# cyrillefavreau/Sol-R

Hardware: AMD Instinct MI355X
Metric: Mrays/s @1920x1080, 3-bounce Cornell (higher is better)
Workload: dtype f32; 1 GPU; cornell 1920x1080, 3 bounces + shadow rays, 75 boxes / 29 primitives, one GPU, whole frame; rays_per_frame=6518779, closest_hit_walks_rank0=3506171, lane_nodes=206382796, lane_prim_tests=37557299, wave_nodes=3396811, wave_prim_tests=626627, wave_walks=106204, cost_ordered_launch_rank0=True, frames_in_flight=3, setup_frames_before_warmup=48, frames_delivered=9105, order_free_nodes=46, short_ray_lists=1, gather=none (one GPU), strips=equal rows, parallelism=tile1

## Files before the change

### sol-r_amd/csrc/engine.h

```cpp
#ifndef SOLR_ENGINE_H
#define SOLR_ENGINE_H

#include <hip/hip_runtime.h>

#include <atomic>
#include <chrono>
#include <cstdio>
#include <cstdlib>
#include <cstring>
#include <string>
#include <vector>

#include "../../include/solr_hip.h"
#include "renderer.h"
#include "lists_device.h"
#include "list_builders.h"

namespace solreng
{
struct HostProfile
{
    const bool on = getenv("SOLR_HIP_HOST_PROFILE") != nullptr;
    struct Entry
    {
// ... 165 lines not shown
    unsigned *hostStats = nullptr;
    unsigned *hostStatsDev = nullptr;
    long key[6] = {0, 0, 0, 0, 0, 0};
    int frames = 0;
    bool reorder = false;
    bool orderValid = false;
    BandCuts orderCuts = {};
    void reset()
    {
        frames = 0;
        reorder = false;
        orderValid = false;
    }
    void release();
};

enum Variant
{
    VARIANT_AUTOMATIC = 0,
    VARIANT_EXACT_LIST = 3,
    VARIANT_ALL_FEATURES = 4,
    VARIANT_NO_GROUPING = 5,
    VARIANT_NO_ORDER_FREE = 6,
    VARIANT_STACK_IN_LDS = 7,
    VARIANT_REFERENCE_LEAVES = 8,
    VARIANT_AO_FIXED_STRIDE = 9,
    VARIANT_NAN_DEEP_STACK = 10,
    VARIANT_UNSORTED_LISTS = 12,
    VARIANT_NO_BAND_WORDS = 13,
    VARIANT_ZERO_STREAM_COUNTERS = 14,
    VARIANT_NO_LAMP_CUTOFF = 15,
    VARIANT_ALL_TRIPS = 16,
    VARIANT_UPLOADED_BUILD_BOXES = 17,
    VARIANT_UPLOADED_SPHERE_LEAVES = 18
};

__host__ __device__ inline int primitiveKind(int type, int facts)
{
    if (!(facts & PRIM_FAST0))
        return KIND_GENERAL;
    if (type == ptSphere && !(facts & PRIM_PROCEDURAL))
        return KIND_SPHERE;
    if ((type == ptXYPlane || type == ptYZPlane || type == ptXZPlane) && !(facts & (PRIM_TEXTURED | PRIM_WIRE2)) &&
        !(type == ptYZPlane && (facts & PRIM_EMISSIVE)))
        return type == ptXYPlane ? KIND_PLANE_XY : (type == ptYZPlane ? KIND_PLANE_YZ : KIND_PLANE_XZ);
    if (type == ptTriangle)
        return KIND_TRIANGLE;
    if (type == ptCylinder || type == ptCone)
        return KIND_CYLINDER;
    return KIND_GENERAL;
}
__host__ __device__ inline int primitiveTag(int type, int facts, bool noKinds)
{
    return type | facts | ((noKinds ? (int)KIND_GENERAL : primitiveKind(type, facts)) << PRIM_KIND_SHIFT);
}
inline bool primitiveContained(int type, int facts)
{
    return type == ptTriangle || type == ptCylinder || (type == ptSphere && !(facts & PRIM_PROCEDURAL)) || type == ptXYPlane ||
           type == ptYZPlane || type == ptXZPlane;
}
inline bool primitiveShadowOpaque(int type, int facts)
{
    return !(facts & PRIM_TRANSPARENT) && !(facts & PRIM_TEXTURED) && type != ptCamera;
}
inline int primitiveFeatures(int type, int facts)
{
    int features = (facts & PRIM_TEXTURED) ? F_TEX : 0;
    switch (type)
    {
    case ptSphere:
    case ptEnvironment:
        return features | ((facts & PRIM_PROCEDURAL) ? F_PROC : F_SPHERE);
    case ptCylinder:
    case ptCone:
        return features | F_CYL;
    case ptEllipsoid:
        return features | F_ELL;
    case ptTriangle:
        return features | F_TRI;
    case ptCamera:
        return features | F_PLANE | F_TEX;
    default:
        return features | F_PLANE;
    }
}

struct NodeList
{
    int copies, lists;
    explicit NodeList(int copies_ = 1, int lists_ = 1) : copies(copies_), lists(lists_) {}
    std::vector<float4> rows;
    std::vector<int> start, origin;
    int nb = 0;
    unsigned offRows = 0, offLeaf = 0;
    unsigned offStart = 0;
    int ordered = 0;
    bool tight = false;
    std::vector<int> refitLevels;

    void reset() { *this = NodeList(copies, lists); }
    unsigned nodes() const { return (unsigned)lists * (unsigned)nb; }
    unsigned rowsOf(int list) const { return solrdev::listRows(offRows, (unsigned)nb, (unsigned)list); }
    unsigned offThin() const { return solrdev::listThin(offRows, nodes()); }
    unsigned offSorted() const { return solrdev::listSorted(offRows, nodes()); }
    unsigned layRows(unsigned row)
    {
        offRows = row;
        return row + (unsigned)copies * solrdev::listCopyRows(nodes());
    }
    unsigned layStart(unsigned row)
    {
        offStart = row * 4;
        return row + (nodes() + 3u) / 4u;
    }
    unsigned layLeaf(unsigned row)
    {
        row = (row + 3u) & ~3u;
        offLeaf = row;
        return row + 4u * nodes() + 4u;
    }
};


struct Arena
{
    DeviceBuffer geometry;
    unsigned offPrims = 0, offLights = 0;
    unsigned rowsFixed = 0;
    bool geometryDirty = true;
    bool deviceAhead = false;
    void layOutAgain() { geometryDirty = true; }
};
struct OrderFreeState
{
    int freeCountdown = 0;
    bool freeHostValid = true;
    bool freeDirty = false;
// ... 33 lines not shown
    bool edited = false;
    DeviceBuffer materialSets;
    int nbDeviceMaterialSets = 0;
    bool materialsSet = false;
};
enum MorphSlot
{
    MORPH_SLOT_FIRST = SOLR_MORPH_TRACK_MAX_KEYS,
    MORPH_SLOT_LAST,
    MORPH_SLOTS
};
struct MorphKey
{
    DeviceBuffer planes;
    int nbPrimitives = -1;
};
struct MorphLampAnswer
{
    int slotA, slotB;
    bool moves;
};
struct Morph
{
    MorphKey keys[MORPH_SLOTS];
    int nbTrackKeys = 0;
    std::vector<MorphLampAnswer> lampAnswers;
    long lampChecked = -1;
    DeviceBuffer lampFlag;
    int nbDeviceMorphs = 0;
    int nbDeviceTrackMorphs = 0;
};
struct Scene
{
    NodeList exact = NodeList(1, 1), walk = NodeList(2, 1), orderFree = NodeList(3, solrdev::ORDER_FREE_LISTS);
    std::vector<float4> hostPrims;
    int nbPrimitives = 0;
    DeviceBuffer lamps;
    int nbLamps = 0;
    int nested = 1;
    bool walkEncloses = false;
    OrderFreeState lists;
    Rotation rotation;
    Morph morph;
    long retags = 0;
    Arena arena;

    void newGeometry(int nested_, bool walkEncloses_, int freeCountdown_)
    {
        nested = nested_;
        walkEncloses = walkEncloses_;
        rotation.refitReady = false;
        rotation.exactStale = false;
        rotation.refitPlanPending = true;
        rotation.nbMovable = -1;
        rotation.lampMoved = false;
        rotation.edited = false;
        rotation.materialsSet = false;
        morphKeysDropped();
        arena.deviceAhead = false;
        orderFree.reset();
        lists.freeCountdown = freeCountdown_;
        lists.freeHostValid = true;
        lists.freeDirty = false;
        lists.dropStage(true);
        lists.freeStale = false;
    }
    bool orderFreeDue() { return lists.freeCountdown > 0 && --lists.freeCountdown == 0; }
// ... 538 lines not shown
```

### sol-r_amd/csrc/renderer_kernel.h

```cpp
#ifndef SOLR_RENDERER_KERNEL_H
#define SOLR_RENDERER_KERNEL_H

#include "renderer.h"

using namespace solrdev;

template <int COUNT, int FEAT, bool VOLUME = false>
#ifndef SOLR_GENERIC_WAVES
#define SOLR_GENERIC_WAVES 0
#endif
#ifndef SOLR_WAVES_PER_EU
#define SOLR_WAVES_PER_EU 4
#endif
__global__ __launch_bounds__(WAVE, (SOLR_GENERIC_WAVES && (FEAT & F_TEX)) ? SOLR_GENERIC_WAVES : SOLR_WAVES_PER_EU) void k_standardRenderer(const SceneArgs, const FrameArgs,
                                                           PixelRecord *__restrict__,
                                                           int4 *__restrict__, unsigned char *__restrict__,
                                                           unsigned long long *__restrict__)
{
    extern __shared__ float ldsStack[];
    constexpr int ARGS = FEAT | F_ARGS;
    constexpr int TRACE = (FEAT & (F_TRI | F_TEX)) ? FEAT : ARGS;
    const RendererArgs &A = rendererArgs();
    const FrameArgs &F = A.F;
    const Scene &S = A.scene();
// ... 383 lines not shown
            }
        }
    }
}

template <int FEAT>
__global__ __launch_bounds__(WAVE, SOLR_WAVES_PER_EU) void k_walkBound(const SceneArgs SA, const char *__restrict__ records,
                                                                       unsigned *__restrict__ visits, unsigned *__restrict__ skipped)
{
    extern __shared__ float ldsStack[];
    const Scene S = makeScene(SA);
    const int lane = threadIdx.x;
    const char *slot = records + (size_t)blockIdx.x * SOLR_WALK_SLOT_BYTES;
    const int4 *head = (const int4 *)slot;
    const float4 *rays = (const float4 *)(slot + 16 * (SOLR_WALK_SLOTS + 1));
    const int recorded = __builtin_amdgcn_readfirstlane(head[0].x);
    const int walks = recorded < SOLR_WALK_SLOTS ? recorded : SOLR_WALK_SLOTS;
    unsigned entries = 0;
    int left_out = recorded - walks;
    for (int j = 0; j < walks; ++j)
    {
        const int4 h = head[1 + j];
        const int kind = __builtin_amdgcn_readfirstlane(h.x);
        if (kind == WALK_GENERAL)
        {
            ++left_out;
            continue;
        }
        const float4 a = rays[((size_t)j * 64 + lane) * 2], b = rays[((size_t)j * 64 + lane) * 2 + 1];
        const int doneAfter = __float_as_int(b.w);
        const bool took_part = doneAfter >= 0;
        const WalkRay r = makeWalkRay(V(a.x, a.y, a.z), took_part ? V(b.x, b.y, b.z) : V(1.f, 1.f, 1.f));
        const int order = (FEAT & F_DEEP) ? (__builtin_amdgcn_readfirstlane(h.w) >> 1) & 3 : 0;
        const Scene W = walkList(S, __builtin_amdgcn_readfirstlane(h.y) != 0, __builtin_amdgcn_readfirstlane(h.z),
                                 (__builtin_amdgcn_readfirstlane(h.w) & 1) != 0, order != 0);
        const PackedRay pr = packRay(r);
        const float cutOff = a.w;
        int cursor = took_part ? 0 : SOLR_CURSOR_DONE;
        int cur = 0, visit = 0;
        while (cur < W.nbBoxes)
        {
            if (ballot(cursor != SOLR_CURSOR_DONE) == 0ull)
                break;
            int nbPrimitives;
            bool entered;
            int leaf;
            if ((FEAT & F_DEEP) && order == 1)
                leaf = advanceTidyDeepSorted(W, pr, cutOff, cursor, cur, nbPrimitives, entered);
            else if ((FEAT & F_DEEP) && order == 2)
                leaf = advanceTidyDeepReversed(W, pr, cutOff, cursor, cur, nbPrimitives, entered);
            else
                leaf = advanceTidy<FEAT>(W, pr, cutOff, cursor, cur, nbPrimitives, entered);
            if (leaf < 0)
                break;
            ++visit;
            entries += entered ? 1u : 0u;
            if (doneAfter == visit)
                cursor = SOLR_CURSOR_DONE;
        }
    }
    visits[(size_t)blockIdx.x * WAVE + lane] = entries;
    if (lane == 0 && left_out > 0)
        atomicAdd(skipped, (unsigned)left_out);
}

#endif
```

### sol-r_amd/csrc/rt_device.h

```cpp
#pragma once

#include <hip/hip_runtime.h>
#include "pow_table.h"

#include "../../include/solr_types.h"
#include "scene_layout.h"

namespace solrdev
{
#define SOLR_DEV __device__ __forceinline__

struct v3
{
    float x, y, z;
};

SOLR_DEV v3 V(float x, float y, float z)
{
    v3 r;
    r.x = x;
    r.y = y;
    r.z = z;
    return r;
}
// ... 837 lines not shown
#define SOLR_NOW() __builtin_readcyclecounter()
#else
#define SOLR_T(...)
#endif

template <int COUNT>
SOLR_DEV void countAdd(unsigned int &c, unsigned int v)
{
    if (COUNT == 1)
        c += v;
}

SOLR_DEV int waveMinInt(int v)
{
#pragma unroll
    for (int off = 32; off > 0; off >>= 1)
    {
        int o = __shfl_xor(v, off, 64);
        v = o < v ? o : v;
    }
    return v;
}

#define SOLR_CURSOR_DONE 0x7fffffff

#define SOLR_WALK_SLOTS 16
#define SOLR_WALK_SLOT_BYTES (16 * (SOLR_WALK_SLOTS + 1) + SOLR_WALK_SLOTS * 64 * 32)
enum WalkKind
{
    WALK_CLOSEST = 0,
    WALK_SHADOW = 1,
    WALK_GENERAL = 2
};
SOLR_DEV void recordWalk(Counters &cnt, int kind, bool freeList, int octant, bool took_part, const WalkRay &r, float cutOff,
                         int doneAfter, bool tight = false, int order = 0)
{
    const unsigned j = cnt.ordinal++;
    if (j >= SOLR_WALK_SLOTS || !cnt.record)
        return;
    const int lane = (int)threadIdx.x & 63;
    float4 *lanes = (float4 *)(cnt.record + 16 * (SOLR_WALK_SLOTS + 1)) + ((size_t)j * 64 + lane) * 2;
    lanes[0] = make_float4(r.o.x, r.o.y, r.o.z, cutOff);
    lanes[1] = make_float4(r.d.x, r.d.y, r.d.z, __int_as_float(took_part ? doneAfter : -1));
    if (lane == 0)
        ((int4 *)cnt.record)[1 + j] = make_int4(kind, freeList ? 1 : 0, octant, (tight ? 1 : 0) | (order << 1));
}

template <int FEAT>
SOLR_DEV bool extendedGeometry(const SceneInfo &si);
struct PrimRec
{
    Row2 head;
    float4 c, d;
    int pi;
    bool packed;
};
SOLR_DEV bool planeClass(int type)
{
    return !(type == ptSphere || type == ptEnvironment || type == ptCylinder || type == ptCone || type == ptEllipsoid ||
             type == ptTriangle);
}
SOLR_DEV v3 recP1(const Scene &S, const PrimRec &r) { return r.packed ? V4(r.c) : V4(primRow(S, r.pi, ROW_P1_INDEX)); }
SOLR_DEV v3 recP2(const Scene &S, const PrimRec &r) { return r.packed ? V4(r.d) : V4(primRow(S, r.pi, ROW_P2)); }
SOLR_DEV v3 recPlaneNormal(const Scene &S, const PrimRec &r) { return r.packed ? V4(r.c) : V4(primRow(S, r.pi, ROW_N0)); }
SOLR_DEV float recPlaneAverage(const Scene &S, const PrimRec &r) { return r.packed ? r.d.x : primRow(S, r.pi, ROW_P2).w; }
SOLR_DEV int recIndex(const Scene &S, const PrimRec &r)
// ... 788 lines not shown
        return 0.f;
    const Scene S = again<FEAT>(S_);
    const SceneInfo si = again<FEAT>(si_);
    SOLR_T(const unsigned long long tw0 = SOLR_NOW();)
    WalkRay r = makeWalkRay(origin, lampCenter - origin);
    r.o = origin + r.dn * si.rayEpsilon;
    const float minDistance = (iteration < 2) ? si.viewDistance : si.viewDistance / (iteration + 1);
    const float lengthOL = length(r.d);
    if (active)
        countAdd<COUNT>(cnt.shadow, 1);
    countAdd<COUNT>(cnt.wShadow, 1);

    const bool fastBoxes = S.orderedBoxes && (ballot(active && !finiteRay(r)) == 0ull);
    const bool tidy = COUNT != 1 && fastBoxes && S.nested;
    const bool freeOrder = tidy && S.nbBoxesFree > 0 && (S.opaqueShadows & SHADOWS_OPAQUE) &&
                           ballot(active && !(longRay(r.d) && minDistance >= 2.f)) == 0ull;
    const bool lampCut = tidy && !freeOrder && (S.opaqueShadows & SHADOWS_LAMP_CUTOFF);
    float farFree = 0.f;
    int octant = 0;
    bool reversed = false;
    if (freeOrder)
    {
        const int signs = ((r.d.x < 0.f ? 1 : 0) | (r.d.y < 0.f ? 2 : 0) | (r.d.z < 0.f ? 4 : 0)) ^ 7;
        const int lane = (int)__builtin_ctzll(ballot(active));
        octant = __builtin_amdgcn_readlane(signs, lane);
        reversed = (FEAT & F_DEEP) && S.sortedLists && ballot(active && signs != octant) == 0ull;
    }
    if (freeOrder || lampCut)
        farFree = 1.0002f + 1.0e-4f * (fabsf(r.o.x) + fabsf(r.o.y) + fabsf(r.o.z)) / lengthOL;
    const float farOrdered =
        (lampCut && longRay(r.d) && minDistance >= 2.f) ? fminf(minDistance, farFree) : minDistance;
    const bool tight = (FEAT & F_PLANE) && tidy && S.tightLists && ballot(active && !tightRay(r, si)) == 0ull;
    reversed = reversed && !tight;
    const Scene W = walkList(S, freeOrder, octant, tight, reversed);
    const int nbBoxes = W.nbBoxes;
    const PackedRay pr = packRay(r);
    int cursor = (active && result < si.shadowIntensity) ? 0 : SOLR_CURSOR_DONE;
    const bool walked = cursor != SOLR_CURSOR_DONE;
    int visit = 0, doneAfter = SOLR_CURSOR_DONE;
    int cur = 0;
    Row2 node;
    node.a = node.b = make_float4(0.f, 0.f, 0.f, 0.f);
    if (!tidy)
        node = boxNode(S, 0);
    while (cur < nbBoxes)
    {
        if (ballot(cursor != SOLR_CURSOR_DONE) == 0ull)
            break;
        int leaf = cur, nbPrimitives;
        bool entered;
        SOLR_T(unsigned long long ta = SOLR_NOW();)
        if (tidy)
        {
            if ((FEAT & F_DEEP) && reversed)
            {
                leaf = advanceTidyDeepReversed(W, pr, farFree, cursor, cur, nbPrimitives, entered);
                leaf = leaf < 0 ? leaf : leaf >> 5;
            }
            else
                leaf = advanceTidy<FEAT>(W, pr, freeOrder ? farFree : farOrdered, cursor, cur, nbPrimitives, entered);
            SOLR_T(const unsigned long long tb = SOLR_NOW(); cnt.tNode += tb - ta; ++cnt.nAdvance; ta = tb;)
            if (leaf < 0)
                break;
        }
        else if (!stepGeneral<COUNT>(S, r, fastBoxes, minDistance, cursor, cur, node, nbPrimitives, entered, cnt) ||
                 nbPrimitives <= 0)
            continue;
// ... 95 lines not shown
            if (hit)
            {
                const float l = length(h.intersection - r.o);
                if (l > si.geometryEpsilon && l < lengthOL)
                {
                    float ratio = h.shadowIntensity * si.shadowIntensity;
                    if (tag & PRIM_TRANSPARENT)
                    {
                        const MaterialHot mh = loadMaterialHot(S, uniform(asint(head.b.w)));
                        v3 O_L = r.dn;
                        float a = fabsf(dot(O_L, h.normal));
                        float rr = (mh.transparency == 0.f) ? 1.f : (1.f - mh.transparency);
                        ratio *= rr * a;
                        color.x += ratio * (0.3f - 0.3f * mh.color.x);
                        color.y += ratio * (0.3f - 0.3f * mh.color.y);
                        color.z += ratio * (0.3f - 0.3f * mh.color.z);
                    }
                    result += ratio;
                }
            }
        }
        if (COUNT == 2)
            ++visit;
        if (cursor != SOLR_CURSOR_DONE && !(result < si.shadowIntensity))
        {
            cursor = SOLR_CURSOR_DONE;
            if (COUNT == 2)
                doneAfter = visit;
        }
        SOLR_T(cnt.tLeaf += SOLR_NOW() - ta; ++cnt.nLeaf;)
    }
    if (COUNT == 2)
        recordWalk(cnt, tidy ? WALK_SHADOW : WALK_GENERAL, freeOrder, octant, walked, r, freeOrder ? farFree : farOrdered,
                   doneAfter, tight, reversed ? 2 : 0);
    result = fmaxf(0.f, fminf(result, si.shadowIntensity));
    SOLR_T(cnt.tShadow += SOLR_NOW() - tw0;)
    return result;
}


SOLR_DEV float rnd(const Scene &S, long i)
{
    return (i >= 0 && i < S.nbRandoms) ? S.randoms[i] : 0.f;
}

template <int FEAT>
SOLR_DEV float4 intersectionShader(const Scene &S, const SceneInfo &si, int pi, int type, int materialId,
                                   const MaterialHot &mh, v3 intersection, v3 areas, const TexOut &o)
{
    float4 c = mh.color;
    c.w = 0.f;
    const bool textured = (FEAT & F_TEX) && mh.ids.x != TEXTURE_NONE;
    if (si.extendedGeometry)
    {
        switch (type)
        {
        case ptCone:
        case ptCylinder:
        case ptEnvironment:
        case ptSphere:
        case ptEllipsoid:
            if (textured)
            {
                const v3 p0 = V4(primRow(S, pi, ROW_P0_TYPE));
                const float vt1x = primRow(S, pi, ROW_N2).w;
                const float vt1y = primRow(S, pi, ROW_UV).x;
                c = sphereUVMapping(p0, vt1x, vt1y, mh.color, loadMaterialCold(S, materialId), S.textures, intersection, o);
// ... 961 lines not shown
```

### sol-r_amd/csrc/scene_layout.h

```cpp
#pragma once

#include <hip/hip_runtime.h>

namespace solrdev
{
struct alignas(16) MaterialHot
{
    float4 innerIllumination;
    float4 color;
    float4 specular;
    float reflection, refraction, transparency, opacity;
    int4 attributes;
    int4 ids;
};
static_assert(sizeof(MaterialHot) == 96, "MaterialHot");

struct alignas(16) MaterialCold
{
    int4 textureMapping;
    int4 textureOffset;
    int4 textureIds;
    int4 advancedTextureOffset;
    int4 advancedTextureIds;
    float2 mappingOffset;
// ... 23 lines not shown
    PRIM_TEXTURED = 1 << 15,
    PRIM_WIDTH_SHIFT = 16,
    PRIM_KIND_SHIFT = 24
};

enum PrimKind
{
    KIND_GENERAL = 0,
    KIND_SPHERE = 1,
    KIND_PLANE_XY = 2,
    KIND_PLANE_YZ = 3,
    KIND_PLANE_XZ = 4,
    KIND_TRIANGLE = 5,
    KIND_CYLINDER = 6
};

enum PrimRow
{
    ROW_P0_TYPE = 0,
    ROW_SIZE_MAT = 1,
    ROW_P1_INDEX = 2,
    ROW_P2 = 3,
    ROW_N0 = 4,
    ROW_N1 = 5,
    ROW_N2 = 6,
    ROW_UV = 7,
    PRIM_ROWS = 8
};

enum ShadowFacts
{
    SHADOWS_OPAQUE = 1,
    SHADOWS_LAMP_CUTOFF = 2,
    SHADOWS_ALL_TRIPS = 4
};

struct SceneArgs
{
    const void *geometry;
    const void *materials;
    const void *textures;
    const void *randoms;
    unsigned offBoxes, offBoxStart, offPrims, offLights, offMatCold;
    int nbBoxes;
    int nbPrimitives;
    int nbLights;
    int nbLamps;
    int nested;
    int orderedBoxes;
    long nbRandoms;
    unsigned offLeaf;
    unsigned offBoxesFree, offLeafFree;
    int nbBoxesFree;
    int opaqueShadows;
    int shortRayLists;
    int tightLists;
    int sortedLists;
};

const int ORDER_FREE_LISTS = 8;
__host__ __device__ constexpr unsigned listCopyRows(unsigned nodes) { return 2u * nodes + 2u; }
__host__ __device__ constexpr unsigned listRows(unsigned offRows, unsigned nb, unsigned list) { return offRows + 2u * (list * nb); }
__host__ __device__ constexpr unsigned listThin(unsigned offRows, unsigned nodes) { return offRows + listCopyRows(nodes); }
__host__ __device__ constexpr unsigned listSorted(unsigned offRows, unsigned nodes) { return offRows + 2u * listCopyRows(nodes); }
__host__ __device__ constexpr unsigned listLeaf(unsigned offLeaf, unsigned nb, unsigned list) { return offLeaf + 4u * (list * nb); }

#define SOLR_CONST_AS __attribute__((address_space(4)))
typedef float f4v __attribute__((ext_vector_type(4)));
typedef int i4v __attribute__((ext_vector_type(4)));
typedef const SOLR_CONST_AS f4v *cf4p;
typedef const SOLR_CONST_AS i4v *ci4p;
typedef const SOLR_CONST_AS int *cip;
typedef const SOLR_CONST_AS float *cfp;
typedef const SOLR_CONST_AS unsigned char *cbp;

struct Scene
{
    cf4p geo;
    cf4p mat;
    cbp textures;
    cfp randoms;
    unsigned offBoxes, offBoxStart, offPrims, offLights, offMatCold;
    int nbBoxes;
    int nbPrimitives;
    int nbLights;
    int nbLamps;
    int nested;
    int orderedBoxes;
    long nbRandoms;
    unsigned offLeaf;
    unsigned offBoxesFree, offLeafFree;
    int nbBoxesFree;
    int opaqueShadows;
    int shortRayLists;
    int tightLists;
    int sortedLists;
};
// ... 18 lines not shown
    s.orderedBoxes = a.orderedBoxes;
    s.nbRandoms = a.nbRandoms;
    s.offLeaf = a.offLeaf;
    s.offBoxesFree = a.offBoxesFree;
    s.offLeafFree = a.offLeafFree;
    s.nbBoxesFree = a.nbBoxesFree;
    s.opaqueShadows = a.opaqueShadows;
    s.shortRayLists = a.shortRayLists;
    s.tightLists = a.tightLists;
    s.sortedLists = a.sortedLists;
    return s;
}

__device__ __forceinline__ Scene walkList(const Scene &S, bool freeList, int octant, bool thin, bool sorted)
{
    Scene W = S;
    unsigned nodes = (unsigned)S.nbBoxes;
    if (freeList)
    {
        nodes = (unsigned)ORDER_FREE_LISTS * (unsigned)S.nbBoxesFree;
        W.offBoxes = listRows(S.offBoxesFree, (unsigned)S.nbBoxesFree, (unsigned)octant);
        W.offLeaf = listLeaf(S.offLeafFree, (unsigned)S.nbBoxesFree, (unsigned)octant);
        W.nbBoxes = S.nbBoxesFree;
    }
    if (freeList && sorted)
    {
        W.offBoxes = listSorted(W.offBoxes, nodes);
        W.nbBoxes = S.nbBoxesFree << 5;
    }
    else if (thin)
        W.offBoxes = listThin(W.offBoxes, nodes);
    return W;
}

typedef float f8v __attribute__((ext_vector_type(8)));
typedef const SOLR_CONST_AS f8v *cf8p;
typedef const SOLR_CONST_AS char *ccp;

__device__ __forceinline__ float4 ld4(cf4p p, unsigned row)
{
    const f4v v = *(cf4p)((ccp)p + (row << 4));
    return make_float4(v.x, v.y, v.z, v.w);
}
struct Row2
{
    float4 a, b;
};
__device__ __forceinline__ Row2 ld8(cf4p p, unsigned row)
{
    const f8v v = *(cf8p)((ccp)p + (row << 4));
    Row2 r;
    r.a = make_float4(v[0], v[1], v[2], v[3]);
    r.b = make_float4(v[4], v[5], v[6], v[7]);
    return r;
}
struct Row4
{
    float4 a, b, c, d;
};
typedef float f16v __attribute__((ext_vector_type(16)));
typedef const SOLR_CONST_AS f16v *cf16p;
__device__ __forceinline__ Row4 ld16(cf4p p, unsigned row)
{
    const f16v v = *(cf16p)((ccp)p + (row << 4));
    Row4 r;
    r.a = make_float4(v[0], v[1], v[2], v[3]);
// ... 68 lines not shown
```

### sol-r_amd/csrc/solr_arena.hip

```cpp
#include <hip/hip_runtime.h>

#include <cmath>

#include "../../include/solr_hip.h"
#include "rt_device.h"

using namespace solrdev;

#include "renderer.h"
#include "engine.h"

using namespace solreng;

namespace solreng
{
__global__ __launch_bounds__(256) void k_buildLeafRecords(float4 *__restrict__ arena, unsigned offNodes, unsigned offStart,
                                                         unsigned offPrims, unsigned offLeaf, int nbNodes)
{
    const int i = blockIdx.x * blockDim.x + threadIdx.x;
    if (i >= nbNodes)
        return;
    float4 r0 = make_float4(0.f, 0.f, 0.f, 0.f), r1 = r0, r2 = r0, r3 = r0;
    const int nb = __float_as_int(arena[offNodes + 2u * (unsigned)i + 1u].z);
    if (nb > 0)
// ... 14 lines not shown
    }
    float4 *out = arena + offLeaf + 4u * (unsigned)i;
    out[0] = r0;
    out[1] = r1;
    out[2] = r2;
    out[3] = r3;
}

__global__ __launch_bounds__(256) void k_tightenLeaves(float4 *__restrict__ arena, unsigned offNodes, unsigned offTight,
                                                      unsigned offStart, unsigned offPrims, int nbNodes, float margin, float reach)
{
    const int i = blockIdx.x * blockDim.x + threadIdx.x;
    if (i >= nbNodes)
        return;
    float4 row0 = arena[offNodes + 2u * (unsigned)i], row1 = arena[offNodes + 2u * (unsigned)i + 1u];
    const int nb = __float_as_int(row1.z);
    if (nb > 0)
    {
        static_assert(BB_KIND_SHIFT == PRIM_KIND_SHIFT && BB_KIND_PLANE_XY == KIND_PLANE_XY && BB_KIND_PLANE_YZ == KIND_PLANE_YZ &&
                          BB_KIND_PLANE_XZ == KIND_PLANE_XZ && BB_KIND_SPHERE == KIND_SPHERE && ROW_P0_TYPE == 0 && ROW_SIZE_MAT == 1,
                      "build_bounds.h reads the primitive records as scene_layout.h lays them out");
        const int start = ((const int *)arena)[offStart + (unsigned)i];
        float lo[3], hi[3];
        if (leafBuildBounds(row0, row1, arena + offPrims, start, nb, margin, lo, hi, true, reach))
        {
            row0 = make_float4(lo[0], lo[1], lo[2], hi[2]);
            row1 = make_float4(hi[0], hi[1], row1.z, row1.w);
        }
    }
    arena[offTight + 2u * (unsigned)i] = row0;
    arena[offTight + 2u * (unsigned)i + 1u] = row1;
}

__global__ __launch_bounds__(256) void k_tightenInner(float4 *__restrict__ arena, unsigned offTight, int nbNodes, int listLength)
{
    const int i = blockIdx.x * blockDim.x + threadIdx.x;
    if (i >= nbNodes)
        return;
    const float4 row0 = arena[offTight + 2u * (unsigned)i], row1 = arena[offTight + 2u * (unsigned)i + 1u];
    const int nb = __float_as_int(row1.z), skip = __float_as_int(row1.w);
    if (nb > 0 || skip <= 1)
        return;
    const int listEnd = (i / listLength + 1) * listLength;
    const int end = min(i + skip, listEnd);
    float lx = INFINITY, ly = INFINITY, lz = INFINITY, hx = -INFINITY, hy = -INFINITY, hz = -INFINITY;
    for (int j = i + 1; j < end; ++j)
    {
        const float4 b = arena[offTight + 2u * (unsigned)j + 1u];
        if (__float_as_int(b.z) <= 0)
            continue;
        const float4 a = arena[offTight + 2u * (unsigned)j];
        lx = fminf(lx, a.x), ly = fminf(ly, a.y), lz = fminf(lz, a.z);
        hx = fmaxf(hx, b.x), hy = fmaxf(hy, b.y), hz = fmaxf(hz, a.w);
    }
    const float nlx = fmaxf(row0.x, lx), nly = fmaxf(row0.y, ly), nlz = fmaxf(row0.z, lz);
    const float nhx = fminf(row1.x, hx), nhy = fminf(row1.y, hy), nhz = fminf(row0.w, hz);
    if (!(nlx <= nhx && nly <= nhy && nlz <= nhz))
        return;
    arena[offTight + 2u * (unsigned)i] = make_float4(nlx, nly, nlz, nhz);
    arena[offTight + 2u * (unsigned)i + 1u] = make_float4(nhx, nhy, row1.z, row1.w);
}

__global__ __launch_bounds__(256) void k_listEncloses(const float4 *__restrict__ arena, unsigned offNodes, unsigned offStart,
                                                      unsigned offPrims, int nbNodes, int nbPrims, int *bad)
{
    const int i = blockIdx.x * blockDim.x + threadIdx.x;
    if (i >= nbNodes)
        return;
    const float4 a = arena[offNodes + 2u * (unsigned)i], b = arena[offNodes + 2u * (unsigned)i + 1u];
    const int count = __float_as_int(b.z);
    const int end = min(i + max(__float_as_int(b.w), 1), nbNodes);
    bool encloses = true;
    if (count <= 0)
    {
        for (int j = i + 1; j < end && encloses;)
        {
            const float4 ca = arena[offNodes + 2u * (unsigned)j], cb = arena[offNodes + 2u * (unsigned)j + 1u];
            encloses = ca.x >= a.x && ca.y >= a.y && ca.z >= a.z && cb.x <= b.x && cb.y <= b.y && ca.w <= a.w;
            j += max(__float_as_int(cb.w), 1);
        }
    }
    else
    {
        const int start = ((const int *)arena)[offStart + (unsigned)i];
        for (int k = 0; k < count && encloses; ++k)
        {
            const long long pi = (long long)start + k;
            if (start < 0 || pi >= nbPrims)
            {
                encloses = false;
                break;
            }
            const float4 *r = arena + offPrims + (size_t)PRIM_ROWS * (size_t)pi;
// ... 52 lines not shown
                       hipMemcpyDeviceToHost));
    if (g.scene.lists.freeStage.origin)
        HIPCHECK(hipMemcpy(list.origin.data(), g.scene.lists.freeStage.origin, n * 4, hipMemcpyDeviceToHost));
    if (ok())
    {
        g.scene.hostListsPulled();
    }
}

void pullGeometry()
{
    if (!g.scene.arena.deviceAhead || !g.scene.arena.geometry.ptr)
        return;
    refreshExactList();
    quiesce();
    auto get = [&](unsigned at, void *dst, size_t bytes) {
        if (bytes)
            HIPCHECK(hipMemcpy(dst, (const char *)g.scene.arena.geometry.ptr + (size_t)at * 16, bytes, hipMemcpyDeviceToHost));
    };
    for (NodeList *list : {&g.scene.exact, &g.scene.walk, &g.scene.orderFree})
        if (list != &g.scene.orderFree || g.scene.lists.freeHostValid)
            get(list->offRows, list->rows.data(), list->rows.size() * 16);
    get(g.scene.arena.offPrims, g.scene.hostPrims.data(), g.scene.hostPrims.size() * 16);
    g.scene.hostImagesPulled();
}

float thinReachWanted(float viewDistance)
{
    if (g.variant == VARIANT_UPLOADED_SPHERE_LEAVES)
        return 0.f;
    return viewDistance > g.facts.sceneExtent ? viewDistance : g.facts.sceneExtent;
}

static bool tightenList(const NodeList &list)
{
    static const bool off = getenv("SOLR_HIP_NO_TIGHT_LEAVES") != nullptr;
    const int nbNodes = (int)list.nodes(), listLength = list.nb;
    const bool worth = g.facts.plainPlanes || (g.facts.looseSpheres && (g.facts.sceneFeatures & F_PLANE) != 0);
    if (off || !worth || nbNodes <= 0 || listLength <= 0 || listLength > 65536 || !ok())
        return false;
    float4 *arena = (float4 *)g.scene.arena.geometry.ptr;
    const float margin = g.facts.sceneExtent * (1.f / 1024.f);
    const dim3 grid((unsigned)((nbNodes + 255) / 256));
    hipLaunchKernelGGL(k_tightenLeaves, grid, dim3(256), 0, sceneStream(), arena, list.offRows, list.offThin(), list.offStart, g.scene.arena.offPrims,
                       nbNodes, margin, g.facts.thinReach);
    hipLaunchKernelGGL(k_tightenInner, grid, dim3(256), 0, sceneStream(), arena, list.offThin(), nbNodes, listLength);
    HIPCHECK(hipGetLastError());
    return ok();
}

__global__ __launch_bounds__(256) void k_sortNodeBounds(float4 *__restrict__ arena, unsigned offBoxesFree, unsigned offSorted, int nb)
{
    const int i = blockIdx.x * blockDim.x + threadIdx.x;
    if (i > 8 * nb)
        return;
    float4 a = make_float4(0.f, 0.f, 0.f, 0.f), b = a;
    if (i < 8 * nb)
    {
        const int octant = i / nb;
        a = arena[offBoxesFree + 2u * (unsigned)i];
        b = arena[offBoxesFree + 2u * (unsigned)i + 1u];
        if (octant & 1)
        {
            const float t = a.x;
            a.x = b.x;
            b.x = t;
        }
        if (octant & 2)
        {
            const float t = a.y;
            a.y = b.y;
            b.y = t;
        }
        if (octant & 4)
        {
            const float t = a.z;
            a.z = a.w;
            a.w = t;
        }
        b.w = __int_as_float(__float_as_int(b.w) << 5);
    }
    arena[offSorted + 2u * (unsigned)i] = a;
    arena[offSorted + 2u * (unsigned)i + 1u] = b;
}

static bool sortFreeLists()
{
    static const bool off = getenv("SOLR_HIP_NO_SORTED_LISTS") != nullptr;
    const NodeList &list = g.scene.orderFree;
    if (off || list.nb <= 0 || !ok())
        return false;
    hipLaunchKernelGGL(k_sortNodeBounds, dim3((unsigned)((8 * list.nb + 1 + 255) / 256)), dim3(256), 0, sceneStream(),
                       (float4 *)g.scene.arena.geometry.ptr, list.offRows, list.offSorted(), list.nb);
    HIPCHECK(hipGetLastError());
    return ok();
}

static void deriveList(NodeList &list)
{
    const bool orderFree = &list == &g.scene.orderFree;
    const int n = (orderFree && g.scene.lists.freeStale) ? 0 : (int)list.nodes();
    if (n > 0)
        hipLaunchKernelGGL(k_buildLeafRecords, dim3((unsigned)((n + 255) / 256)), dim3(256), 0, sceneStream(), (float4 *)g.scene.arena.geometry.ptr,
                           list.offRows, list.offStart, g.scene.arena.offPrims, list.offLeaf, n);
    HIPCHECK(hipGetLastError());
    list.tight = list.copies > 1 && n > 0 && tightenList(list);
    if (orderFree)
        g.scene.lists.sortedFree = n > 0 && sortFreeLists();
}

void buildLeafRecords()
{
    if (!ok() || !g.scene.arena.geometry.ptr)
        return;
    for (NodeList *list : {&g.scene.exact, &g.scene.walk, &g.scene.orderFree})
        deriveList(*list);
    HIPCHECK(hipStreamSynchronize(sceneStream()));
}

void tightenListsAgain()
{
    if (!ok() || !g.scene.arena.geometry.ptr)
        return;
    for (NodeList *list : {&g.scene.walk, &g.scene.orderFree})
        if (list->tight)
            list->tight = tightenList(*list);
    HIPCHECK(hipStreamSynchronize(sceneStream()));
}

static void copyStagedLists()
{
    const NodeList &list = g.scene.orderFree;
    char *arena = (char *)g.scene.arena.geometry.ptr;
    const SolrDeviceLists &stage = g.scene.lists.freeStage;
    HIPCHECK(hipMemcpyAsync(arena + (size_t)list.offRows * 16, stage.rows, (size_t)list.nodes() * 32, hipMemcpyDeviceToDevice, sceneStream()));
    HIPCHECK(hipMemcpyAsync(arena + (size_t)list.offStart * 4, stage.start, (size_t)list.nodes() * 4, hipMemcpyDeviceToDevice, sceneStream()));
}

static void appendFreeLists()
// ... 195 lines not shown
    {
        if (origin.empty())
            ownOrigins();
        count = buildFreeOrderLists(rows, start, origin, built.rows, built.start, built.origin, &prunedFree, knobs.pruneThreshold,
                                    pruneDecider(), build);
    }
    if (getenv("SOLR_HIP_DEBUG_TREE"))
        fprintf(stderr, "solr_hip: order-free lists: 8 x %d nodes (%d inner nodes that hardly cull left out)\n", count, prunedFree);
    if (count <= 0)
        return;
    phase.mark("order-free: tree, pruning, eight flattenings");
    built.nb = count;
    g.scene.orderFreeBuilt(built, stayed, fromArena);
}

bool orderFreeListsUsable()
{
    return g.scene.orderFree.nb > 0 && g.facts.primsContained && !g.scene.lists.freeStale && g.scene.nested && g.scene.walk.ordered &&
           g.variant != VARIANT_NO_ORDER_FREE;
}

bool lampCutoffUsable()
{
    return g.scene.walkEncloses && g.facts.primsContained && g.scene.nested && g.scene.walk.ordered && g.variant != VARIANT_NO_LAMP_CUTOFF;
}

static int tightListsFor(const SceneArgs &S, const SceneInfo &sceneInfo, bool exactNodes)
{
    if (exactNodes || g.variant == VARIANT_REFERENCE_LEAVES || !g.scene.walk.tight || !g.scene.walkEncloses || !sceneInfo.extendedGeometry)
        return 0;
    if (S.nbBoxesFree > 0 && !g.scene.orderFree.tight)
        return 0;
    return (sceneInfo.viewDistance > 0.f && sceneInfo.viewDistance <= 64.f * g.facts.sceneExtent) ? 1 : 0;
}

static bool sortedListsUsable(int nbBoxesFree)
{
    return nbBoxesFree > 0 && g.scene.lists.sortedFree && g.variant != VARIANT_UNSORTED_LISTS;
}

bool shortRayListsChoice()
{
    static const int fromEnv = getenv("SOLR_HIP_SHORT_RAY_LISTS") ? atoi(getenv("SOLR_HIP_SHORT_RAY_LISTS")) : -1;
    const int mode = g.shortRayListsMode >= 0 ? g.shortRayListsMode : fromEnv;
    return mode < 0 ? activeFlights() >= 2 : mode != 0;
}

static SceneArgs makeScene(bool exactNodes)
{
    const NodeList &list = exactNodes ? g.scene.exact : g.scene.walk;
    SceneArgs S;
    memset(&S, 0, sizeof(S));
    S.geometry = g.scene.arena.geometry.ptr;
    S.materials = g.materials.table.ptr;
    S.textures = g.textures.atlas.ptr;
    S.randoms = g.randoms.values.ptr;
    S.offBoxes = list.offRows;
    S.offBoxStart = list.offStart;
    S.offLeaf = list.offLeaf;
    S.offPrims = g.scene.arena.offPrims;
    S.offLights = g.scene.arena.offLights;
    S.offMatCold = g.materials.offMatCold;
    S.nbBoxes = list.nb;
    S.nbPrimitives = g.scene.nbPrimitives;
    S.nbLights = g.lights.nbLights;
    S.nbLamps = g.scene.nbLamps;
    S.nested = g.scene.nested;
    S.orderedBoxes = list.ordered;
    S.nbRandoms = g.randoms.values.ptr ? g.randoms.nbRandoms : 0;
    if (!exactNodes && orderFreeListsUsable())
    {
        S.offBoxesFree = g.scene.orderFree.offRows;
        S.offLeafFree = g.scene.orderFree.offLeaf;
        S.nbBoxesFree = g.scene.orderFree.nb;
        S.opaqueShadows = g.facts.opaqueShadows ? SHADOWS_OPAQUE : 0;
        S.shortRayLists = shortRayListsChoice() ? 1 : 0;
    }
    if (!exactNodes && lampCutoffUsable())
        S.opaqueShadows |= SHADOWS_LAMP_CUTOFF;
    if (g.variant == VARIANT_ALL_TRIPS)
        S.opaqueShadows |= SHADOWS_ALL_TRIPS;
    S.tightLists = 0;
    S.sortedLists = sortedListsUsable(S.nbBoxesFree) ? 1 : 0;
    return S;
}

SceneArgs prepareScene(const SceneInfo &sceneInfo, bool exactNodes)
{
    maybeBuildOrderFreeLists();
    flushGeometry();
    if (exactNodes)
        refreshExactList();
    if (!ok())
        return SceneArgs();
    SceneArgs S = makeScene(exactNodes);
    S.tightLists = tightListsFor(S, sceneInfo, exactNodes);
    g.facts.frameViewDistance = sceneInfo.viewDistance;
    if (S.tightLists && thinReachWanted(sceneInfo.viewDistance) != g.facts.thinReach)
    {
        quiesce();
        g.facts.thinReach = thinReachWanted(sceneInfo.viewDistance);
        tightenListsAgain();
        if (!ok())
            return SceneArgs();
    }
    return S;
}

bool deepNodeList(const SceneArgs &S)
{
    return S.nbBoxes > 1024;
}

}
```

### sol-r_amd/csrc/solr_diag.hip

```cpp
#include <hip/hip_runtime.h>
#include <dlfcn.h>
#include <fcntl.h>
#include <sched.h>
#include <sys/mman.h>
#include <sys/stat.h>
#include <unistd.h>

#include <atomic>

#include <cmath>
#include <cstdio>
#include <cstdlib>
#include <cstring>
#include <string>
#include <functional>
#include <chrono>
#include <vector>

#include "../../include/solr_hip.h"
#include "rt_device.h"
#include "device_pool.h"
#include "lists_device.h"

using namespace solrdev;
// ... 43 lines not shown
    if (!ok())
        return -1;
    const int flight = g.current;
    const hipStream_t stream = g.flight[flight].stream;
    const size_t pixels = (size_t)g.width * g.height;
    HIPCHECK(hipMemcpyAsync(g.flight[flight].pp.ptr, frame, pixels * sizeof(PostProcessingBuffer), hipMemcpyHostToDevice, stream));
    unsigned char *bitmap = (unsigned char *)g.flight[flight].shown().ptr;
    const bool neighbourhood = (ppInfo.type == ppe_ambientOcclusion || ppInfo.type == ppe_depthOfField ||
                                ppInfo.type == ppe_radiosity || ppInfo.type == ppe_filter || ppInfo.type == ppe_cartoon);
    if (neighbourhood)
    {
        HaloDebt nothingOwed;
        launchPostProcess(sceneInfo, ppInfo, flight, stream, 0, g.height, bitmap, nothingOwed);
    }
    else
    {
        solrpost::defaultConversion(stream, sceneInfo, (int)pixels, (const PixelRecord *)g.flight[flight].pp.ptr, bitmap);
        HIPCHECK(hipGetLastError());
    }
    HIPCHECK(hipMemcpyAsync(bitmapOut, bitmap, pixels * SOLR_COLOR_DEPTH, hipMemcpyDeviceToHost, stream));
    HIPCHECK(hipStreamSynchronize(stream));
    return ok() ? 0 : -1;
}

void lastFrame(int out[6])
{
    memcpy(out, g.lastFrame, sizeof(g.lastFrame));
}

int listCopy(int list, int what, void *out, int capacity)
{
    if (!ready("solr_hip_probe_list_copy"))
        return -1;
    ARGCHECK(list >= 0 && list <= 2 && what >= 0 && what <= 4, "solr_hip_probe_list_copy: no such list or copy");
    ARGCHECK(g.scene.arena.geometry.ptr != nullptr || g.scene.arena.geometryDirty, "solr_hip_probe_list_copy: no scene uploaded");
    if (!ok())
        return -1;
    HIPCHECK(hipSetDevice(g.device));
    flushGeometry();
    if (list == 1)
        refreshExactList();
    quiesce();
    if (!ok() || !g.scene.arena.geometry.ptr)
        return -1;
    const NodeList &L = list == 0 ? g.scene.walk : (list == 1 ? g.scene.exact : g.scene.orderFree);
    const unsigned nodes = (list == 2 && g.scene.lists.freeStale) ? 0u : L.nodes();
    size_t at = 0, count = 0, unit = 16;
    switch (what)
    {
    case 0:
        at = (size_t)L.offRows * 16, count = 2 * (size_t)nodes;
        break;
    case 1:
        at = (size_t)L.offThin() * 16, count = (L.copies > 1 && L.tight) ? 2 * (size_t)nodes : 0;
        break;
    case 2:
        at = (size_t)L.offSorted() * 16, count = (list == 2 && L.copies > 2 && g.scene.lists.sortedFree) ? 2 * (size_t)nodes + 2 : 0;
        break;
    case 3:
        at = (size_t)L.offLeaf * 16, count = 4 * (size_t)nodes;
        break;
    default:
        at = (size_t)L.offStart * 4, count = nodes, unit = 4;
        break;
    }
    if (nodes == 0)
        count = 0;
    if (!out)
        return (int)count;
    ARGCHECK(count <= (size_t)(capacity < 0 ? 0 : capacity), "solr_hip_probe_list_copy: capacity too small");
    ARGCHECK(at + count * unit <= g.scene.arena.geometry.bytes, "solr_hip_probe_list_copy: the copy lies outside the arena");
    if (!ok())
        return -1;
    if (count)
        HIPCHECK(hipMemcpy(out, (const char *)g.scene.arena.geometry.ptr + at, count * unit, hipMemcpyDeviceToHost));
    return ok() ? (int)count : -1;
}

int walkOffer(const SceneInfo &sceneInfo, bool exactNodes, int out[8])
{
    SceneArgs S;
    int features, deep;
    hipStream_t stream;
    if (residentScene(sceneInfo, exactNodes, &S, &features, &deep, &stream) != 0)
        return -1;
    const float margin = g.facts.sceneExtent * (1.f / 1024.f), extent = g.facts.sceneExtent;
    out[0] = S.tightLists, out[1] = S.sortedLists, out[2] = S.nbBoxesFree, out[3] = S.opaqueShadows, out[4] = S.shortRayLists;
    out[5] = S.nbBoxes;
    memcpy(&out[6], &margin, 4);
    memcpy(&out[7], &extent, 4);
    return 0;
}
}
// ... 401 lines not shown
```

Baseline: 31750 Mrays/s.

## Add shadow-only walk list that leaves out lamp-only leaves for shadow rays

Builds a third copy of the walk node list in which leaves that contain only the single lamp primitive get bounds pushed far away, and inner boxes are re-tightened around what remains. Shadow rays toward that lamp, when tight lists apply and the whole wave targets it, walk this copy, so they no longer enter the lamp's leaf and test its primitives. The replay path in the renderer picks up the same copy through a new walk flag. This costs an extra node-list copy in the arena plus two more build kernels, and correctness depends on the lamp never occluding its own shadow rays.

```diff
diff --git a/sol-r_amd/csrc/engine.h b/sol-r_amd/csrc/engine.h
--- a/sol-r_amd/csrc/engine.h
+++ b/sol-r_amd/csrc/engine.h
@@ -221,7 +221,8 @@
     VARIANT_NO_LAMP_CUTOFF = 15,
     VARIANT_ALL_TRIPS = 16,
     VARIANT_UPLOADED_BUILD_BOXES = 17,
-    VARIANT_UPLOADED_SPHERE_LEAVES = 18
+    VARIANT_UPLOADED_SPHERE_LEAVES = 18,
+    VARIANT_SHADOWS_ENTER_LAMP = 19
 };
 
 __host__ __device__ inline int primitiveKind(int type, int facts)
@@ -285,6 +286,7 @@
     unsigned offStart = 0;
     int ordered = 0;
     bool tight = false;
+    int shadowLamp = -1;
     std::vector<int> refitLevels;
 
     void reset() { *this = NodeList(copies, lists); }
@@ -292,6 +294,7 @@
     unsigned rowsOf(int list) const { return solrdev::listRows(offRows, (unsigned)nb, (unsigned)list); }
     unsigned offThin() const { return solrdev::listThin(offRows, nodes()); }
     unsigned offSorted() const { return solrdev::listSorted(offRows, nodes()); }
+    unsigned offShadow() const { return solrdev::listShadow(offRows, nodes()); }
     unsigned layRows(unsigned row)
     {
         offRows = row;
@@ -391,7 +394,7 @@
 };
 struct Scene
 {
-    NodeList exact = NodeList(1, 1), walk = NodeList(2, 1), orderFree = NodeList(3, solrdev::ORDER_FREE_LISTS);
+    NodeList exact = NodeList(1, 1), walk = NodeList(3, 1), orderFree = NodeList(3, solrdev::ORDER_FREE_LISTS);
     std::vector<float4> hostPrims;
     int nbPrimitives = 0;
     DeviceBuffer lamps;
diff --git a/sol-r_amd/csrc/renderer_kernel.h b/sol-r_amd/csrc/renderer_kernel.h
--- a/sol-r_amd/csrc/renderer_kernel.h
+++ b/sol-r_amd/csrc/renderer_kernel.h
@@ -439,8 +439,11 @@
         const bool took_part = doneAfter >= 0;
         const WalkRay r = makeWalkRay(V(a.x, a.y, a.z), took_part ? V(b.x, b.y, b.z) : V(1.f, 1.f, 1.f));
         const int order = (FEAT & F_DEEP) ? (__builtin_amdgcn_readfirstlane(h.w) >> 1) & 3 : 0;
-        const Scene W = walkList(S, __builtin_amdgcn_readfirstlane(h.y) != 0, __builtin_amdgcn_readfirstlane(h.z),
-                                 (__builtin_amdgcn_readfirstlane(h.w) & 1) != 0, order != 0);
+        Scene W = walkList(S, __builtin_amdgcn_readfirstlane(h.y) != 0, __builtin_amdgcn_readfirstlane(h.z),
+                           (__builtin_amdgcn_readfirstlane(h.w) & 1) != 0, order != 0);
+        if ((FEAT & F_PLANE) && (__builtin_amdgcn_readfirstlane(h.w) & (WALK_SHADOW_COPY | 1)) == (WALK_SHADOW_COPY | 1) &&
+            __builtin_amdgcn_readfirstlane(h.y) == 0)
+            W.offBoxes = shadowList(S).offBoxes;
         const PackedRay pr = packRay(r);
         const float cutOff = a.w;
         int cursor = took_part ? 0 : SOLR_CURSOR_DONE;
diff --git a/sol-r_amd/csrc/rt_device.h b/sol-r_amd/csrc/rt_device.h
--- a/sol-r_amd/csrc/rt_device.h
+++ b/sol-r_amd/csrc/rt_device.h
@@ -893,6 +893,7 @@
     WALK_SHADOW = 1,
     WALK_GENERAL = 2
 };
+#define WALK_SHADOW_COPY 8
 SOLR_DEV void recordWalk(Counters &cnt, int kind, bool freeList, int octant, bool took_part, const WalkRay &r, float cutOff,
                          int doneAfter, bool tight = false, int order = 0)
 {
@@ -1747,7 +1748,11 @@
         (lampCut && longRay(r.d) && minDistance >= 2.f) ? fminf(minDistance, farFree) : minDistance;
     const bool tight = (FEAT & F_PLANE) && tidy && S.tightLists && ballot(active && !tightRay(r, si)) == 0ull;
     reversed = reversed && !tight;
-    const Scene W = walkList(S, freeOrder, octant, tight, reversed);
+    const bool lampLeafOut = (FEAT & F_PLANE) && tight && !freeOrder && (S.opaqueShadows & SHADOWS_LAMP_LEAF_OUT) &&
+                             ballot(active && lightId != (S.opaqueShadows >> SHADOWS_LAMP_SHIFT)) == 0ull;
+    Scene W = walkList(S, freeOrder, octant, tight, reversed);
+    if (lampLeafOut)
+        W.offBoxes = shadowList(S).offBoxes;
     const int nbBoxes = W.nbBoxes;
     const PackedRay pr = packRay(r);
     int cursor = (active && result < si.shadowIntensity) ? 0 : SOLR_CURSOR_DONE;
@@ -1909,7 +1914,7 @@
     }
     if (COUNT == 2)
         recordWalk(cnt, tidy ? WALK_SHADOW : WALK_GENERAL, freeOrder, octant, walked, r, freeOrder ? farFree : farOrdered,
-                   doneAfter, tight, reversed ? 2 : 0);
+                   doneAfter, tight, (reversed ? 2 : 0) | (lampLeafOut ? WALK_SHADOW_COPY >> 1 : 0));
     result = fmaxf(0.f, fminf(result, si.shadowIntensity));
     SOLR_T(cnt.tShadow += SOLR_NOW() - tw0;)
     return result;
diff --git a/sol-r_amd/csrc/scene_layout.h b/sol-r_amd/csrc/scene_layout.h
--- a/sol-r_amd/csrc/scene_layout.h
+++ b/sol-r_amd/csrc/scene_layout.h
@@ -79,7 +79,10 @@
 {
     SHADOWS_OPAQUE = 1,
     SHADOWS_LAMP_CUTOFF = 2,
-    SHADOWS_ALL_TRIPS = 4
+    SHADOWS_ALL_TRIPS = 4,
+    SHADOWS_LAMP_LEAF_OUT = 8,
+    SHADOWS_LAMP_SHIFT = 8,
+    SHADOWS_LAMP_LIMIT = 1 << 22
 };
 
 struct SceneArgs
@@ -110,6 +113,7 @@
 __host__ __device__ constexpr unsigned listRows(unsigned offRows, unsigned nb, unsigned list) { return offRows + 2u * (list * nb); }
 __host__ __device__ constexpr unsigned listThin(unsigned offRows, unsigned nodes) { return offRows + listCopyRows(nodes); }
 __host__ __device__ constexpr unsigned listSorted(unsigned offRows, unsigned nodes) { return offRows + 2u * listCopyRows(nodes); }
+__host__ __device__ constexpr unsigned listShadow(unsigned offRows, unsigned nodes) { return offRows + 2u * listCopyRows(nodes); }
 __host__ __device__ constexpr unsigned listLeaf(unsigned offLeaf, unsigned nb, unsigned list) { return offLeaf + 4u * (list * nb); }
 
 #define SOLR_CONST_AS __attribute__((address_space(4)))
@@ -194,6 +198,12 @@
         W.offBoxes = listThin(W.offBoxes, nodes);
     return W;
 }
+__device__ __forceinline__ Scene shadowList(const Scene &S)
+{
+    Scene W = S;
+    W.offBoxes = listShadow(S.offBoxes, (unsigned)S.nbBoxes);
+    return W;
+}
 
 typedef float f8v __attribute__((ext_vector_type(8)));
 typedef const SOLR_CONST_AS f8v *cf8p;
diff --git a/sol-r_amd/csrc/solr_arena.hip b/sol-r_amd/csrc/solr_arena.hip
--- a/sol-r_amd/csrc/solr_arena.hip
+++ b/sol-r_amd/csrc/solr_arena.hip
@@ -70,7 +70,8 @@
     arena[offTight + 2u * (unsigned)i + 1u] = row1;
 }
 
-__global__ __launch_bounds__(256) void k_tightenInner(float4 *__restrict__ arena, unsigned offTight, int nbNodes, int listLength)
+#define SHADOW_OUT_AT 0x1p99f
+__global__ __launch_bounds__(256) void k_tightenInner(float4 *__restrict__ arena, unsigned offTight, int nbNodes, int listLength, bool leaveOut)
 {
     const int i = blockIdx.x * blockDim.x + threadIdx.x;
     if (i >= nbNodes)
@@ -88,6 +89,8 @@
         if (__float_as_int(b.z) <= 0)
             continue;
         const float4 a = arena[offTight + 2u * (unsigned)j];
+        if (leaveOut && a.x >= SHADOW_OUT_AT)
+            continue;
         lx = fminf(lx, a.x), ly = fminf(ly, a.y), lz = fminf(lz, a.z);
         hx = fmaxf(hx, b.x), hy = fmaxf(hy, b.y), hz = fmaxf(hz, a.w);
     }
@@ -97,6 +100,31 @@
         return;
     arena[offTight + 2u * (unsigned)i] = make_float4(nlx, nly, nlz, nhz);
     arena[offTight + 2u * (unsigned)i + 1u] = make_float4(nhx, nhy, row1.z, row1.w);
+}
+
+#define SHADOW_VIEW_LIMIT 0x1p57f
+__global__ __launch_bounds__(256) void k_shadowLeaves(float4 *__restrict__ arena, unsigned offTight, unsigned offShadow, unsigned offStart,
+                                                     unsigned offPrims, int nbNodes, int nbPrims, int lampIndex)
+{
+    const int i = blockIdx.x * blockDim.x + threadIdx.x;
+    if (i >= nbNodes)
+        return;
+    float4 row0 = arena[offTight + 2u * (unsigned)i], row1 = arena[offTight + 2u * (unsigned)i + 1u];
+    const int nb = __float_as_int(row1.z);
+    if (nb > 0)
+    {
+        const int start = ((const int *)arena)[offStart + (unsigned)i];
+        bool lampOnly = start >= 0 && (long long)start + nb <= (long long)nbPrims;
+        for (int k = 0; k < nb && lampOnly; ++k)
+            lampOnly = __float_as_int(arena[offPrims + 8u * (unsigned)(start + k) + ROW_P1_INDEX].w) == lampIndex;
+        if (lampOnly)
+        {
+            row0 = make_float4(SHADOW_OUT_AT, SHADOW_OUT_AT, SHADOW_OUT_AT, SHADOW_OUT_AT);
+            row1 = make_float4(SHADOW_OUT_AT, SHADOW_OUT_AT, row1.z, row1.w);
+        }
+    }
+    arena[offShadow + 2u * (unsigned)i] = row0;
+    arena[offShadow + 2u * (unsigned)i + 1u] = row1;
 }
 
 __global__ __launch_bounds__(256) void k_listEncloses(const float4 *__restrict__ arena, unsigned offNodes, unsigned offStart,
@@ -215,8 +243,9 @@
     return viewDistance > g.facts.sceneExtent ? viewDistance : g.facts.sceneExtent;
 }
 
-static bool tightenList(const NodeList &list)
-{
+static bool tightenList(NodeList &list)
+{
+    list.shadowLamp = -1;
     static const bool off = getenv("SOLR_HIP_NO_TIGHT_LEAVES") != nullptr;
     const int nbNodes = (int)list.nodes(), listLength = list.nb;
     const bool worth = g.facts.plainPlanes || (g.facts.looseSpheres && (g.facts.sceneFeatures & F_PLANE) != 0);
@@ -227,8 +256,19 @@
     const dim3 grid((unsigned)((nbNodes + 255) / 256));
     hipLaunchKernelGGL(k_tightenLeaves, grid, dim3(256), 0, sceneStream(), arena, list.offRows, list.offThin(), list.offStart, g.scene.arena.offPrims,
                        nbNodes, margin, g.facts.thinReach);
-    hipLaunchKernelGGL(k_tightenInner, grid, dim3(256), 0, sceneStream(), arena, list.offThin(), nbNodes, listLength);
+    hipLaunchKernelGGL(k_tightenInner, grid, dim3(256), 0, sceneStream(), arena, list.offThin(), nbNodes, listLength, false);
+    const int lamp = (&list == &g.scene.walk && list.copies > 2 && list.lists == 1 && g.lights.nbLights == 1 && g.lights.hostLights.size() >= 3)
+                         ? bitsi(g.lights.hostLights[0].w)
+                         : -1;
+    if (lamp >= 0 && lamp < SHADOWS_LAMP_LIMIT)
+    {
+        hipLaunchKernelGGL(k_shadowLeaves, grid, dim3(256), 0, sceneStream(), arena, list.offThin(), list.offShadow(), list.offStart,
+                           g.scene.arena.offPrims, nbNodes, (int)(g.scene.hostPrims.size() / PRIM_ROWS), lamp);
+        hipLaunchKernelGGL(k_tightenInner, grid, dim3(256), 0, sceneStream(), arena, list.offShadow(), nbNodes, listLength, true);
+    }
     HIPCHECK(hipGetLastError());
+    if (ok() && lamp >= 0 && lamp < SHADOWS_LAMP_LIMIT)
+        list.shadowLamp = lamp;
     return ok();
 }
 
@@ -288,6 +328,8 @@
                            list.offRows, list.offStart, g.scene.arena.offPrims, list.offLeaf, n);
     HIPCHECK(hipGetLastError());
     list.tight = list.copies > 1 && n > 0 && tightenList(list);
+    if (!list.tight)
+        list.shadowLamp = -1;
     if (orderFree)
         g.scene.lists.sortedFree = n > 0 && sortFreeLists();
 }
@@ -549,6 +591,13 @@
     if (S.nbBoxesFree > 0 && !g.scene.orderFree.tight)
         return 0;
     return (sceneInfo.viewDistance > 0.f && sceneInfo.viewDistance <= 64.f * g.facts.sceneExtent) ? 1 : 0;
+}
+
+static int lampLeafOutUsable(int tightLists, const SceneInfo &sceneInfo)
+{
+    if (!tightLists || g.scene.walk.shadowLamp < 0 || g.lights.nbLights != 1 || g.variant == VARIANT_SHADOWS_ENTER_LAMP)
+        return -1;
+    return sceneInfo.viewDistance <= SHADOW_VIEW_LIMIT ? g.scene.walk.shadowLamp : -1;
 }
 
 static bool sortedListsUsable(int nbBoxesFree)
@@ -612,6 +661,9 @@
         return SceneArgs();
     SceneArgs S = makeScene(exactNodes);
     S.tightLists = tightListsFor(S, sceneInfo, exactNodes);
+    const int lampOut = lampLeafOutUsable(S.tightLists, sceneInfo);
+    if (lampOut >= 0)
+        S.opaqueShadows |= SHADOWS_LAMP_LEAF_OUT | (lampOut << SHADOWS_LAMP_SHIFT);
     g.facts.frameViewDistance = sceneInfo.viewDistance;
     if (S.tightLists && thinReachWanted(sceneInfo.viewDistance) != g.facts.thinReach)
     {
diff --git a/sol-r_amd/csrc/solr_diag.hip b/sol-r_amd/csrc/solr_diag.hip
--- a/sol-r_amd/csrc/solr_diag.hip
+++ b/sol-r_amd/csrc/solr_diag.hip
@@ -99,7 +99,7 @@
 {
     if (!ready("solr_hip_probe_list_copy"))
         return -1;
-    ARGCHECK(list >= 0 && list <= 2 && what >= 0 && what <= 4, "solr_hip_probe_list_copy: no such list or copy");
+    ARGCHECK(list >= 0 && list <= 2 && what >= 0 && what <= 5, "solr_hip_probe_list_copy: no such list or copy");
     ARGCHECK(g.scene.arena.geometry.ptr != nullptr || g.scene.arena.geometryDirty, "solr_hip_probe_list_copy: no scene uploaded");
     if (!ok())
         return -1;
@@ -126,6 +126,9 @@
         break;
     case 3:
         at = (size_t)L.offLeaf * 16, count = 4 * (size_t)nodes;
+        break;
+    case 5:
+        at = (size_t)L.offShadow() * 16, count = (list == 0 && L.copies > 2 && L.tight && L.shadowLamp >= 0) ? 2 * (size_t)nodes + 2 : 0;
         break;
     default:
         at = (size_t)L.offStart * 4, count = nodes, unit = 4;
```

New measurement: 32070 Mrays/s (median of 6 runs). Within noise of the previous version (+1.0%).
